# TaceoLabs/co-snarks

Measured on AMD Instinct MI355X. Metric: BN254 G1 MSM points/sec, higher is better.
Workload: dtype i32x9 29-bit-limb lazy Montgomery, i64 accumulate (BN254 Fq 254-bit); 1 GPU; BN254 G1 Pippenger MSM, uniform scalars / known-dlog points, 2^20 points per GPU (BASELINE config 2); points_total=1048576, points_per_gpu=1048576, split=single GPU, exchange_mode=none, rccl_ranks_seen=0, spinup_steps=190

## Files before the change

co-snarks_amd/csrc/curve_quad.hpp:

```cpp
#pragma once
#include <stddef.h>

#include "curve_lazy.hpp"

namespace csh {

#if defined(__HIP_DEVICE_COMPILE__) || defined(__HIPCC__)

template <int P0, int P1, int P2, int P3>
struct QuadCtrl {
  static constexpr int value = P0 | (P1 << 2) | (P2 << 4) | (P3 << 6);
};

template <int CTRL>
__device__ __forceinline__ int32_t quad_mov(int32_t v) {
  return __builtin_amdgcn_mov_dpp(v, CTRL, 0xf, 0xf, true);
}

template <int CTRL, class LP, class F32>
__device__ __forceinline__ FpS<LP, F32> quad_perm(const FpS<LP, F32>& a) {
  FpS<LP, F32> r;
#pragma unroll
  for (int i = 0; i < FpS<LP, F32>::NL; ++i) r.l[i] = quad_mov<CTRL>(a.l[i]);
  return r;
// ... 41 lines not shown
  (&p->x)[role] = q.v;
  if (role == 0) p->empty = q.empty;
}
static_assert(offsetof(XYZZLazy<Fq29s>, y) == sizeof(Fq29s) && offsetof(XYZZLazy<Fq29s>, zzz) == 3 * sizeof(Fq29s), "XYZZLazy members must be contiguous");

template <int SRC>
__device__ __forceinline__ bool quad_bcast_flag(bool f) {
  return quad_mov<QuadCtrl<SRC, SRC, SRC, SRC>::value>((int32_t)f) != 0;
}

template <class L>
__device__ __forceinline__ void qdbl(QPt<L>& acc, int role) {
  if (acc.empty) return;
  if (quad_bcast_flag<1>(acc.v.maybe_zero())) {
    if (quad_bcast_flag<1>(acc.v.is_zero_slow())) {
      acc = qpt_inf<L>();
      return;
    }
  }
  const L U = L::add(acc.v, acc.v).normalized();
  const L A = lane_select(role == 1, U, acc.v);
  const L SQ = L::sqr(A);
  const L V = quad_perm<QBcast1::value>(SQ);
  const L R2 = L::mul(A, V);
  const L M = L::add(L::add(SQ, SQ), SQ).normalized();
  const L W = quad_perm<QBcast1::value>(R2);
  const L R3 = L::mul(lane_select(role == 0, M, acc.v), lane_select(role == 0, M, W));
  const L x3 = L::sub(R3, L::add(R2, R2)).normalized();
  const L T = L::sub(R2, x3);
  const L Mb = quad_perm<QBcast0::value>(M);
  const L Tb = quad_perm<QBcast0::value>(T);
  const L y3 = L::mul_sub(Mb, Tb, R2, acc.v);
  acc.v = role == 0 ? x3 : (role == 1 ? y3 : (role == 2 ? R2 : R3));
}

template <class L>
__device__ __forceinline__ void qadd(QPt<L>& acc, const QPt<L>& p, int role) {
  if (p.empty) return;
  if (acc.empty) {
    acc = p;
    return;
  }
  const L R1 = L::mul(acc.v, quad_perm<QZzOwn::value>(p.v));
  const L R2 = L::mul(p.v, quad_perm<QZzOwn::value>(acc.v));
  const L D = L::sub(R2, R1);
  if (quad_bcast_flag<0>(D.maybe_zero())) {
    if (quad_bcast_flag<0>(D.is_zero_slow())) {
      if (quad_bcast_flag<1>(D.is_zero())) {
        qdbl<L>(acc, role);
      } else {
        acc = qpt_inf<L>();
      }
      return;
    }
  }
  const L SQ = L::sqr(D);
  const L pp = quad_perm<QBcast0::value>(SQ);
  const L pb = quad_perm<QBcast0::value>(D);
  const L R4 = L::mul(lane_select(role == 3, pb, R1), pp);
  const L ppp = quad_perm<QBcast3::value>(R4);
  const L rr = quad_perm<QBcast1::value>(SQ);
  const L x3 = L::sub(L::sub(rr, ppp), L::add(R4, R4)).normalized();
  const L T = quad_perm<QBcast0::value>(L::sub(R4, x3));
  const L a = lane_select(role == 1, D, R1);
  const L b = lane_select(role == 1, T, R4);
  const L c = lane_select(role == 1, R1, L::zero());
  const L R5 = L::mul_sub(a, b, c, ppp);
  acc.v = role == 0 ? x3 : (role == 2 ? R4 : R5);
}

template <class L>
__device__ __forceinline__ QPt<L> qmul_small(const QPt<L>& p, uint32_t k, int role) {
  QPt<L> r = qpt_inf<L>();
  if (k == 0 || p.empty) return r;
  int top = 31;
  while (!((k >> top) & 1)) --top;
  for (int b = top; b >= 0; --b) {
    qdbl<L>(r, role);
    if ((k >> b) & 1) qadd<L>(r, p, role);
  }
  return r;
}

#endif

}
```

co-snarks_amd/csrc/host_fp64.hpp:

```cpp
#pragma once
#include <stdint.h>
#include <string.h>

#include "field.hpp"

namespace csh {

template <class P>
struct Fp64 {
  static_assert(P::N % 2 == 0, "limb count must be even");
  static constexpr int N = P::N / 2;
  using Params = P;
  uint64_t l[N];

  static uint64_t word(const uint32_t* w, int i) { return (uint64_t)w[2 * i] | ((uint64_t)w[2 * i + 1] << 32); }
  static uint64_t inv64() {
    static const uint64_t v = [] {
      const uint64_t p0 = word(P::MOD, 0);
      uint64_t y = p0;
      for (int i = 0; i < 6; ++i) y *= 2 - p0 * y;
      return (uint64_t)0 - y;
    }();
    return v;
  }
  static Fp64 zero() {
    Fp64 r;
    for (int i = 0; i < N; ++i) r.l[i] = 0;
    return r;
  }
  static Fp64 one() {
    Fp64 r;
    for (int i = 0; i < N; ++i) r.l[i] = word(P::R1, i);
    return r;
  }
  bool is_zero() const {
    uint64_t a = 0;
    for (int i = 0; i < N; ++i) a |= l[i];
    return a == 0;
  }
  bool operator==(const Fp64& b) const { return memcmp(l, b.l, sizeof l) == 0; }
  bool operator!=(const Fp64& b) const { return !(*this == b); }

  static bool geq_mod(const uint64_t* a) {
    for (int i = N - 1; i >= 0; --i) {
      const uint64_t m = word(P::MOD, i);
      if (a[i] > m) return true;
      if (a[i] < m) return false;
    }
    return true;
  }
  static void sub_mod(uint64_t* a) {
    unsigned __int128 br = 0;
    for (int i = 0; i < N; ++i) {
      const unsigned __int128 d = (unsigned __int128)a[i] - word(P::MOD, i) - (uint64_t)br;
      a[i] = (uint64_t)d;
      br = (d >> 64) & 1;
    }
  }
  static Fp64 add(const Fp64& a, const Fp64& b) {
    Fp64 r;
    unsigned __int128 c = 0;
    for (int i = 0; i < N; ++i) {
      c += (unsigned __int128)a.l[i] + b.l[i];
      r.l[i] = (uint64_t)c;
      c >>= 64;
    }
    if (geq_mod(r.l)) sub_mod(r.l);
    return r;
  }
  static Fp64 sub(const Fp64& a, const Fp64& b) {
    Fp64 r;
    uint64_t br = 0;
    for (int i = 0; i < N; ++i) {
      const unsigned __int128 d = (unsigned __int128)a.l[i] - b.l[i] - br;
      r.l[i] = (uint64_t)d;
      br = (uint64_t)(d >> 64) & 1;
    }
    if (br) {
      unsigned __int128 c = 0;
      for (int i = 0; i < N; ++i) {
        c += (unsigned __int128)r.l[i] + word(P::MOD, i);
        r.l[i] = (uint64_t)c;
        c >>= 64;
      }
    }
    return r;
  }
  static Fp64 neg(const Fp64& a) { return a.is_zero() ? a : sub(zero(), a); }
  static Fp64 mul(const Fp64& a, const Fp64& b) {
    uint64_t t[N + 2];
    for (int i = 0; i < N + 2; ++i) t[i] = 0;
    const uint64_t inv = inv64();
    for (int i = 0; i < N; ++i) {
      unsigned __int128 c = 0;
      for (int j = 0; j < N; ++j) {
        c += (unsigned __int128)a.l[j] * b.l[i] + t[j];
        t[j] = (uint64_t)c;
        c >>= 64;
      }
      c += t[N];
      t[N] = (uint64_t)c;
      t[N + 1] = (uint64_t)(c >> 64);
      const uint64_t m = t[0] * inv;
      c = (unsigned __int128)m * word(P::MOD, 0) + t[0];
      c >>= 64;
      for (int j = 1; j < N; ++j) {
        c += (unsigned __int128)m * word(P::MOD, j) + t[j];
        t[j - 1] = (uint64_t)c;
        c >>= 64;
      }
      c += t[N];
      t[N - 1] = (uint64_t)c;
      t[N] = t[N + 1] + (uint64_t)(c >> 64);
    }
    Fp64 r;
    for (int i = 0; i < N; ++i) r.l[i] = t[i];
    if (t[N] || geq_mod(r.l)) sub_mod(r.l);
    return r;
  }
  static Fp64 sqr(const Fp64& a) { return mul(a, a); }
  static Fp64 mul2(const Fp64& a) { return add(a, a); }
  static Fp64 mul3(const Fp64& a) { return add(add(a, a), a); }
  static Fp64 mul4(const Fp64& a) { return mul2(mul2(a)); }
  static Fp64 mul8(const Fp64& a) { return mul2(mul4(a)); }
  static Fp64 inv(const Fp64& a) {
    Fp64 r = one();
    for (int i = P::N * 32 - 1; i >= 0; --i) {
      r = sqr(r);
      if ((P::PM2[i >> 5] >> (i & 31)) & 1) r = mul(r, a);
    }
    return r;
  }
};

template <class F>
struct Host64;
template <class P>
struct Host64<Fp<P>> {
  using type = Fp64<P>;
};
template <class P, int NR>
struct Host64<Fp2T<Fp<P>, NR>> {
  using type = Fp2T<Fp64<P>, NR>;
};

}
```

co-snarks_amd/csrc/msm_impl.hpp:

```cpp
#pragma once
#include <stdlib.h>
#include <string.h>

#include <algorithm>
#include <type_traits>
#include <vector>

#include "common.hpp"
#include "curve.hpp"
#include "curve_lazy.hpp"
#include "curve_quad.hpp"
#include "curve_pair.hpp"
#include "host_fp64.hpp"
#include "msm_digits.hpp"
#include "msm_plan.hpp"
#include "msm_sort.hpp"
#include "msm_sort_wide.hpp"


namespace csh {

struct Bn254G1Cfg { using Fq = Bn254Fq;   using Fr = Bn254Fr; static constexpr bool LAZY = true;  using L = Fq29s; static constexpr bool INLINE_ADD = true; static constexpr bool PAIR = false; };
struct Bn254G2Cfg { using Fq = Bn254Fq2;  using Fr = Bn254Fr; static constexpr bool LAZY = true;  using L = Fq29s2; static constexpr bool INLINE_ADD = true; static constexpr bool PAIR = true; static constexpr bool PAIR_ACC_DEFAULT = false; using LP = Fp2Pair<Fq29s>; };
struct Bls381G1Cfg { using Fq = Bls381Fq;  using Fr = Bls381Fr; static constexpr bool LAZY = true;  using L = Fq28s; static constexpr bool INLINE_ADD = true; static constexpr bool PAIR = false; };
// ... 117 lines not shown
          if (pos + 2 < hi) e_next2 = so[pos + 2];
        } else {
          e_next = so[pos + 1];
          pt_next = bases[e_next & 0x7fffffffu];
        }
      }
      const bool inf = stored_is_inf(pt);
      const L x = L::unpack(pt.x);
      const L y = L::unpack(pt.y).cneg_unpacked(e >> 31);
      if (pos == next) {
        pw[b + k] = acc;
        do { ++b; next = st[b + 1]; } while (next <= pos);
        acc.x = x;
        acc.y = y;
        acc.zz = L::one();
        acc.zzz = L::one();
        acc.empty = inf;
        continue;
      }
      if (inf) continue;
      lazy_madd<L, Affine<Fq>>(acc, x, y, bases + (e & 0x7fffffffu), e >> 31);
    }
    pw[b + k] = acc;
  }
}

template <class Cfg>
__global__ __launch_bounds__(ACC_BLK) void k_msm_accum_pair(const Affine<typename Cfg::Fq>* __restrict__ bases, MsmParams p,
                                                            const uint32_t* __restrict__ start, const uint32_t* __restrict__ nlanes,
                                                            const uint32_t* __restrict__ sorted, LazyPt<Cfg>* partial, uint32_t* giant_count) {
  using Fq = typename Cfg::Fq;
  using L = typename Cfg::LP;
  using LF = typename L::Base;
  using F32 = decltype(bases->x.c0);
  const int w = blockIdx.y;
  const int role = pair_role();
  const uint32_t k = (blockIdx.x * blockDim.x + threadIdx.x) >> 1;
  if (blockIdx.x == 0 && threadIdx.x == 0 && w == 0) {
    giant_count[0] = 0;
    giant_count[1] = 0;
  }
  if (k >= nlanes[w]) return;
  const uint32_t* st = start + (size_t)w * (p.NB + 2);
  const uint32_t total = st[p.NB + 1];
  const uint32_t Lw = lane_len(p, w);
  const uint32_t lo = k * Lw;
  uint32_t hi = lo + Lw;
  if (hi > total) hi = total;
  uint32_t b = upper_bound_u32(st, 1, p.NB + 1, lo) - 1;
  uint32_t next = st[b + 1];
  const uint32_t* so = sorted + (size_t)w * p.n;
  LazyPt<Cfg>* pw = partial + (size_t)w * p.tmax;
  const F32* half = reinterpret_cast<const F32*>(bases) + role;
  XYZZLazy<L> acc = XYZZLazy<L>::inf();
  uint32_t e_next = so[lo];
  F32 x_next = half[4 * (size_t)(e_next & 0x7fffffffu)], y_next = half[4 * (size_t)(e_next & 0x7fffffffu) + 2];
  for (uint32_t pos = lo; pos < hi; ++pos) {
    const uint32_t e = e_next;
    const F32 xs = x_next, ys = y_next;
    if (pos + 1 < hi) {
      e_next = so[pos + 1];
      x_next = half[4 * (size_t)(e_next & 0x7fffffffu)];
      y_next = half[4 * (size_t)(e_next & 0x7fffffffu) + 2];
    }
    const bool inf = pair_all((top_word(xs) | top_word(ys)) == 0 && xs.is_zero() && ys.is_zero());
    const L x{LF::unpack(xs)};
    const L y{LF::unpack(ys).cneg_unpacked(e >> 31)};
    if (pos == next) {
      pair_store(&pw[b + k], role, acc);
      do { ++b; next = st[b + 1]; } while (next <= pos);
      acc.x = x;
      acc.y = y;
      acc.zz = L::one();
      acc.zzz = L::one();
      acc.empty = inf;
      continue;
    }
    if (inf) continue;
    lazy_madd<L, Affine<Fq>>(acc, x, y, bases + (e & 0x7fffffffu), e >> 31);
  }
  pair_store(&pw[b + k], role, acc);
}

constexpr int TAIL_BLK = 64;
constexpr int TAIL_Q = TAIL_BLK / 4;

constexpr uint32_t MERGE_CAP = 16;
constexpr uint32_t GIANT_BIG = 256, GIANT_SLICES = 16, GIANT_BIG_CAP = 128, GIANT_ROWS = 32, GIANT_SLICED_FLAG = 0x80000000u;
__device__ __forceinline__ void giant_enqueue(uint32_t* giant_count, uint32_t* giant_list, uint32_t* big_list, uint32_t w, uint32_t b, uint32_t nparts) {
  uint32_t tag = w;
  if (nparts >= GIANT_BIG) {
    const uint32_t q = atomicAdd(giant_count + 1, 1u);
    if (q < GIANT_BIG_CAP) {
      big_list[2 * q] = w;
      big_list[2 * q + 1] = b;
      tag |= GIANT_SLICED_FLAG;
    }
  }
  const uint32_t g = atomicAdd(giant_count, 1u);
  giant_list[2 * g] = tag;
  giant_list[2 * g + 1] = b;
}
template <class Cfg>
__global__ __launch_bounds__(TAIL_BLK) void k_msm_merge(MsmParams p, const uint32_t* __restrict__ start,
                                                        const LazyPt<Cfg>* __restrict__ partial, LazyPt<Cfg>* dense,
                                                        uint32_t* giant_count, uint32_t* giant_list, uint32_t* big_list) {
  using L = typename Cfg::L;
  const int w = blockIdx.y;
  const int role = threadIdx.x & 3;
  const uint32_t b = blockIdx.x * TAIL_Q + (threadIdx.x >> 2) + 1;
  if (b > p.NB) return;
  const uint32_t* st = start + (size_t)w * (p.NB + 2);
  const uint32_t lo = st[b], hi = st[b + 1];
  QPt<L> acc = qpt_inf<L>();
  if (hi > lo) {
    const uint32_t Lw = lane_len(p, w);
    const uint32_t k0 = lo / Lw, k1 = (hi - 1) / Lw;
    const LazyPt<Cfg>* pw = partial + (size_t)w * p.tmax + b;
    if (k1 - k0 >= MERGE_CAP) {
      if (role == 0) giant_enqueue(giant_count, giant_list, big_list, (uint32_t)w, b, k1 - k0 + 1);
    } else {
      acc = qpt_load<L>(&pw[k0], role);
      for (uint32_t k = k0 + 1; k <= k1; ++k) qadd<L>(acc, qpt_load<L>(&pw[k], role), role);
    }
  }
  qpt_store<L>(&dense[(size_t)w * (p.NB + 1) + b], role, acc);
}

template <class L>
__device__ __forceinline__ void quad_block_tree(QPt<L>& x, XYZZLazy<L>* sh, int q, int nq, int role) {
  for (int half = nq >> 1; half >= 1; half >>= 1) {
    if (q >= half && q < 2 * half) qpt_store<L>(&sh[q - half], role, x);
    __syncthreads();
    if (q < half) qadd<L>(x, qpt_load<L>(&sh[q], role), role);
    __syncthreads();
  }
}

template <class Cfg>
__global__ __launch_bounds__(256) void k_msm_giant_slices(MsmParams p, const uint32_t* __restrict__ start, const LazyPt<Cfg>* __restrict__ partial,
                                                          const uint32_t* __restrict__ giant_count, const uint32_t* __restrict__ big_list,
                                                          LazyPt<Cfg>* gscratch) {
  using L = typename Cfg::L;
  __shared__ XYZZLazy<L> sh[32];
  const uint32_t sl = blockIdx.x;
  const uint32_t nbig = giant_count[1] < GIANT_BIG_CAP ? giant_count[1] : GIANT_BIG_CAP;
  const int role = threadIdx.x & 3, qd = threadIdx.x >> 2;
  for (uint32_t q = blockIdx.y; q < nbig; q += gridDim.y) {
    const uint32_t w = big_list[2 * q], b = big_list[2 * q + 1];
    const uint32_t* st = start + (size_t)w * (p.NB + 2);
    const uint32_t Lw = lane_len(p, (int)w);
    const uint32_t k0 = st[b] / Lw, k1 = (st[b + 1] - 1) / Lw;
    const uint32_t per = (k1 - k0 + GIANT_SLICES) / GIANT_SLICES;
    const uint32_t a = k0 + sl * per;
    uint32_t e = a + per;
    if (e > k1 + 1) e = k1 + 1;
    const LazyPt<Cfg>* pw = partial + (size_t)w * p.tmax + b;
    QPt<L> acc = qpt_inf<L>();
    for (uint32_t k = a + qd; k < e; k += 64) qadd<L>(acc, qpt_load<L>(&pw[k], role), role);
    quad_block_tree<L>(acc, sh, qd, 64, role);
    if (qd == 0) qpt_store<L>(&gscratch[(size_t)q * GIANT_SLICES + sl], role, acc);
  }
}

template <class Cfg>
__global__ __launch_bounds__(256) void k_msm_merge_giant(MsmParams p, const uint32_t* __restrict__ start,
                                                         const LazyPt<Cfg>* __restrict__ partial, LazyPt<Cfg>* dense,
                                                         const uint32_t* __restrict__ giant_count, const uint32_t* __restrict__ giant_list,
                                                         const uint32_t* __restrict__ big_list, const LazyPt<Cfg>* __restrict__ gscratch) {
  using L = typename Cfg::L;
  __shared__ XYZZLazy<L> sh[32];
  __shared__ uint32_t slot;
  const uint32_t count = giant_count[0];
  const uint32_t nbig = giant_count[1] < GIANT_BIG_CAP ? giant_count[1] : GIANT_BIG_CAP;
  const int role = threadIdx.x & 3, q = threadIdx.x >> 2;
  for (uint32_t g = blockIdx.x; g < count; g += gridDim.x) {
    const uint32_t tag = giant_list[2 * g], w = tag & ~GIANT_SLICED_FLAG, b = giant_list[2 * g + 1];
    QPt<L> acc = qpt_inf<L>();
    if (tag & GIANT_SLICED_FLAG) {
      __syncthreads();
      if (threadIdx.x == 0) slot = GIANT_BIG_CAP;
      __syncthreads();
      if (threadIdx.x < nbig && big_list[2 * threadIdx.x] == w && big_list[2 * threadIdx.x + 1] == b) slot = threadIdx.x;
      __syncthreads();
      if (slot < GIANT_BIG_CAP) {
        if ((uint32_t)q < GIANT_SLICES) acc = qpt_load<L>(&gscratch[(size_t)slot * GIANT_SLICES + q], role);
      } else {
        const uint32_t* st = start + (size_t)w * (p.NB + 2);
        const uint32_t Lw = lane_len(p, (int)w);
        const uint32_t k0 = st[b] / Lw, k1 = (st[b + 1] - 1) / Lw;
        const LazyPt<Cfg>* pw = partial + (size_t)w * p.tmax + b;
        for (uint32_t k = k0 + q; k <= k1; k += 64) qadd<L>(acc, qpt_load<L>(&pw[k], role), role);
      }
    } else {
      const uint32_t* st = start + (size_t)w * (p.NB + 2);
      const uint32_t Lw = lane_len(p, (int)w);
      const uint32_t k0 = st[b] / Lw, k1 = (st[b + 1] - 1) / Lw;
      const LazyPt<Cfg>* pw = partial + (size_t)w * p.tmax + b;
      for (uint32_t k = k0 + q; k <= k1; k += 64) qadd<L>(acc, qpt_load<L>(&pw[k], role), role);
    }
    quad_block_tree<L>(acc, sh, q, 64, role);
    if (q == 0) qpt_store<L>(&dense[(size_t)w * (p.NB + 1) + b], role, acc);
  }
}

template <class Cfg>
__global__ __launch_bounds__(256) void k_msm_mark_giant(MsmParams p, const uint32_t* __restrict__ start, uint32_t* giant_count, uint32_t* giant_list,
                                                        uint32_t* big_list) {
  const int w = blockIdx.y;
  const uint32_t b = blockIdx.x * 256 + threadIdx.x + 1;
  if (b > p.NB) return;
  const uint32_t* st = start + (size_t)w * (p.NB + 2);
  const uint32_t lo = st[b], hi = st[b + 1];
  const uint32_t Lw = lane_len(p, w);
  if (hi > lo && (hi - 1) / Lw - lo / Lw >= MERGE_CAP) giant_enqueue(giant_count, giant_list, big_list, (uint32_t)w, b, (hi - 1) / Lw - lo / Lw + 1);
}
template <class Cfg>
__device__ __forceinline__ QPt<typename Cfg::L> qbucket_merged(uint32_t Lw, const uint32_t* __restrict__ st, const LazyPt<Cfg>* __restrict__ pw,
                                                               const LazyPt<Cfg>* __restrict__ dw, uint32_t t, int role) {
  using L = typename Cfg::L;
  const uint32_t lo = st[t], hi = st[t + 1];
  if (hi <= lo) return qpt_inf<L>();
  const uint32_t k0 = lo / Lw, k1 = (hi - 1) / Lw;
  if (k1 - k0 >= MERGE_CAP) return qpt_load<L>(&dw[t], role);
  QPt<L> acc = qpt_load<L>(&pw[t + k0], role);
  for (uint32_t k = k0 + 1; k <= k1; ++k) qadd<L>(acc, qpt_load<L>(&pw[t + k], role), role);
  return acc;
}
template <class Cfg>
__device__ __forceinline__ XYZZLazy<typename Cfg::LP> pbucket_merged(uint32_t Lw, const uint32_t* __restrict__ st, const LazyPt<Cfg>* __restrict__ pw,
                                                                     const LazyPt<Cfg>* __restrict__ dw, uint32_t t, int role) {
  using L = typename Cfg::LP;
  const uint32_t lo = st[t], hi = st[t + 1];
  if (hi <= lo) return XYZZLazy<L>::inf();
  const uint32_t k0 = lo / Lw, k1 = (hi - 1) / Lw;
  if (k1 - k0 >= MERGE_CAP) return dw[t].empty ? XYZZLazy<L>::inf() : pair_load(&dw[t], role);
  XYZZLazy<L> acc = pw[t + k0].empty ? XYZZLazy<L>::inf() : pair_load(&pw[t + k0], role);
  for (uint32_t k = k0 + 1; k <= k1; ++k) {
    if (pw[t + k].empty) continue;
    const XYZZLazy<L> q = pair_load(&pw[t + k], role);
    lazy_add_inl<L>(acc, q);
  }
  return acc;
}

template <class Cfg, bool FUSED>
__global__ __launch_bounds__(256) void k_msm_reduce(MsmParams p, const LazyPt<Cfg>* __restrict__ dense,
                                                    LazyPt<Cfg>* segres, const uint32_t* __restrict__ start, const LazyPt<Cfg>* __restrict__ partial) {
  using L = typename Cfg::L;
  const int w = blockIdx.y;
  const int role = threadIdx.x & 3;
  const uint32_t k = blockIdx.x * 64 + (threadIdx.x >> 2);
  if (k >= p.S) return;
  const uint32_t per = (p.NB + p.S - 1) / p.S;
  const uint32_t t0 = 1 + k * per;
  uint32_t t1 = t0 + per;
  if (t1 > p.NB + 1) t1 = p.NB + 1;
  QPt<L> running = qpt_inf<L>(), acc = qpt_inf<L>();
  uint32_t prev_b = 0;
  if (t0 < t1) {
    const LazyPt<Cfg>* dw = dense + (size_t)w * (p.NB + 1);
    const uint32_t* st = FUSED ? start + (size_t)w * (p.NB + 2) : nullptr;
    const LazyPt<Cfg>* pw = FUSED ? partial + (size_t)w * p.tmax : nullptr;
    for (uint32_t t = t1; t-- > t0;) {
      QPt<L> pt;
      if constexpr (FUSED) pt = qbucket_merged<Cfg>(lane_len(p, w), st, pw, dw, t, role);
      else pt = qpt_load<L>(&dw[t], role);
      if (pt.empty) continue;
      uint32_t gap = prev_b ? prev_b - t : 0;
      if (gap) {
        if (gap <= 4) {
          while (gap--) qadd<L>(acc, running, role);
        } else {
          const QPt<L> m = qmul_small<L>(running, gap, role);
          qadd<L>(acc, m, role);
        }
      }
      qadd<L>(running, pt, role);
      prev_b = t;
    }
    if (prev_b) {
      const QPt<L> m = qmul_small<L>(running, prev_b, role);
      qadd<L>(acc, m, role);
    }
  }
  qpt_store<L>(&segres[(size_t)w * p.S + k], role, acc);
}

constexpr int RED_BLK = 256;

template <class Cfg>
__global__ __launch_bounds__(RED_BLK) void k_msm_reduce_serial(MsmParams p, const LazyPt<Cfg>* __restrict__ dense, LazyPt<Cfg>* segres) {
  using L = typename Cfg::L;
  const int w = blockIdx.y;
  const uint32_t k = blockIdx.x * RED_BLK + threadIdx.x;
  if (k >= p.S) return;
  const uint32_t per = (p.NB + p.S - 1) / p.S;
  const uint32_t t0 = 1 + k * per;
  uint32_t t1 = t0 + per;
  if (t1 > p.NB + 1) t1 = p.NB + 1;
  LazyPt<Cfg> running = LazyPt<Cfg>::inf(), acc = LazyPt<Cfg>::inf();
  uint32_t prev_b = 0;
  if (t0 < t1) {
    const LazyPt<Cfg>* dw = dense + (size_t)w * (p.NB + 1);
    for (uint32_t t = t1; t-- > t0;) {
      const LazyPt<Cfg> pt = dw[t];
      if (pt.empty) continue;
      uint32_t gap = prev_b ? prev_b - t : 0;
      if (gap) {
        if (gap <= 4) {
          while (gap--) lazy_add_inl<L>(acc, running);
        } else {
          const LazyPt<Cfg> m = lazy_mul_small<L, true>(running, gap);
          lazy_add_inl<L>(acc, m);
        }
      }
      lazy_add_inl<L>(running, pt);
      prev_b = t;
    }
    if (prev_b) {
      const LazyPt<Cfg> m = lazy_mul_small<L, true>(running, prev_b);
      lazy_add_inl<L>(acc, m);
    }
  }
  segres[(size_t)w * p.S + k] = acc;
}

template <class Cfg, bool FUSED>
__global__ __launch_bounds__(RED_BLK) void k_msm_reduce_pair(MsmParams p, const LazyPt<Cfg>* __restrict__ dense, LazyPt<Cfg>* segres,
                                                             const uint32_t* __restrict__ start, const LazyPt<Cfg>* __restrict__ partial) {
  using L = typename Cfg::LP;
  const int w = blockIdx.y;
  const int role = pair_role();
  const uint32_t k = blockIdx.x * (RED_BLK / 2) + (threadIdx.x >> 1);
  if (k >= p.S) return;
  const uint32_t per = (p.NB + p.S - 1) / p.S;
  const uint32_t t0 = 1 + k * per;
  uint32_t t1 = t0 + per;
  if (t1 > p.NB + 1) t1 = p.NB + 1;
  XYZZLazy<L> running = XYZZLazy<L>::inf(), acc = XYZZLazy<L>::inf();
  uint32_t prev_b = 0;
  if (t0 < t1) {
    const LazyPt<Cfg>* dw = dense + (size_t)w * (p.NB + 1);
    const uint32_t* st = FUSED ? start + (size_t)w * (p.NB + 2) : nullptr;
    const LazyPt<Cfg>* pw = FUSED ? partial + (size_t)w * p.tmax : nullptr;
    for (uint32_t t = t1; t-- > t0;) {
      XYZZLazy<L> pt;
      if constexpr (FUSED) {
        pt = pbucket_merged<Cfg>(lane_len(p, w), st, pw, dw, t, role);
        if (pt.empty) continue;
      } else {
        if (dw[t].empty) continue;
        pt = pair_load(&dw[t], role);
      }
      uint32_t gap = prev_b ? prev_b - t : 0;
      if (gap) {
        if (gap <= 4) {
          while (gap--) lazy_add_inl<L>(acc, running);
        } else {
          const XYZZLazy<L> m = lazy_mul_small<L, true>(running, gap);
          lazy_add_inl<L>(acc, m);
        }
      }
      lazy_add_inl<L>(running, pt);
      prev_b = t;
// ... 146 lines not shown
  CSH_TRY(msm_sort_prepare<Fr>(p, pdig, scalars_dev, st, ar, &ss));
  CSH_TRY(msm_sort_launch(p, ss.sb, st, ev));
  *out = SortOut{ss.sb.start, ss.sb.nlanes, ss.sb.sorted};
  return CSH_OK;
}

template <class Cfg>
struct BucketBufs {
  LazyPt<Cfg>*partial, *segres, *dense, *fold_a, *fold_b;
  uint32_t* giant;
  uint32_t* big;
  LazyPt<Cfg>* gscratch;
  uint32_t fold_n1, max_lanes, max_giant, giant_blocks;
};
constexpr int MAX_GROUPS = 8;
template <class Cfg>
BucketBufs<Cfg> bucket_take(const MsmParams& p, Arena& ar) {
  BucketBufs<Cfg> b;
  b.max_lanes = (uint32_t)(((size_t)p.n + p.L - 1) / p.L);
  b.max_giant = (uint32_t)(((uint64_t)b.max_lanes * p.W) / MERGE_CAP + 1);
  b.giant_blocks = b.max_giant < 1024 ? b.max_giant : 1024;
  b.partial = ar.take<LazyPt<Cfg>>((size_t)p.tmax * p.W);
  b.segres = ar.take<LazyPt<Cfg>>((size_t)p.S * p.W);
  b.dense = ar.take<LazyPt<Cfg>>((size_t)(p.NB + 1) * p.W);
  b.giant = ar.take<uint32_t>((2 * (size_t)b.max_giant + 2) * MAX_GROUPS);
  b.big = ar.take<uint32_t>((size_t)2 * GIANT_BIG_CAP * MAX_GROUPS);
  b.gscratch = ar.take<LazyPt<Cfg>>((size_t)GIANT_BIG_CAP * GIANT_SLICES * MAX_GROUPS);
  b.fold_n1 = (p.S + 127) / 128;
  b.fold_a = ar.take<LazyPt<Cfg>>((size_t)b.fold_n1 * p.W);
  b.fold_b = ar.take<LazyPt<Cfg>>((size_t)b.fold_n1 * p.W);
  return b;
}
template <class Cfg>
size_t msm_bucket_bytes(const MsmParams* pp) {
  Arena sizing;
  bucket_take<Cfg>(*pp, sizing);
  return sizing.off;
}

template <class Cfg>
int bucket_group(const void* points, const MsmParams& p_all, const SortOut& so, const BucketBufs<Cfg>& bb, int w0, int nw, int group, hipStream_t st,
                 void* win_out_dev, hipEvent_t* ev) {
  using Fq = typename Cfg::Fq;
  MsmParams p = p_all;
  p.wide = p_all.wide > w0 ? p_all.wide - w0 : 0;
  const size_t len = (size_t)p.NB + 2;
  const uint32_t* start = so.start + len * w0;
  const uint32_t* nlanes = so.nlanes + w0;
  const uint32_t* sorted = so.sorted + (size_t)p.n * w0;
  LazyPt<Cfg>* partial = bb.partial + (size_t)p.tmax * w0;
  LazyPt<Cfg>* segres = bb.segres + (size_t)p.S * w0;
  LazyPt<Cfg>* dense = bb.dense + (size_t)(p.NB + 1) * w0;
  LazyPt<Cfg>* fold_a = bb.fold_a + (size_t)bb.fold_n1 * w0;
  LazyPt<Cfg>* fold_b = bb.fold_b + (size_t)bb.fold_n1 * w0;
  uint32_t* giant = bb.giant + (2 * (size_t)bb.max_giant + 2) * group;
  uint32_t* big = bb.big + (size_t)2 * GIANT_BIG_CAP * group;
  LazyPt<Cfg>* gscratch = bb.gscratch + (size_t)GIANT_BIG_CAP * GIANT_SLICES * group;
  const Affine<Fq>* bases = reinterpret_cast<const Affine<Fq>*>(points);
  {
    const int tb = tune().acc_blk.load(std::memory_order_relaxed);
    const int blk = (tb == 64 || tb == 128) ? tb : ACC_BLK;
    bool pair = false;
    if constexpr (Cfg::PAIR) pair = Cfg::PAIR_ACC_DEFAULT != ((tune().msm_variant.load(std::memory_order_relaxed) & 2) != 0);
    if constexpr (Cfg::PAIR) {
      if (pair) {
        const dim3 ag((2 * bb.max_lanes + blk - 1) / blk, nw), ab(blk);
        hipLaunchKernelGGL(k_msm_accum_pair<Cfg>, ag, ab, 0, st, bases, p, start, nlanes, sorted, partial, giant);
      }
    }
    if (!pair) {
      const dim3 ag((bb.max_lanes + blk - 1) / blk, nw), ab(blk);
      hipLaunchKernelGGL(k_msm_accum<Cfg>, ag, ab, 0, st, bases, p, start, nlanes, sorted, partial, giant);
    }
  }
  if (ev) CSH_HIP(hipEventRecord(ev[4], st));
  const int variant = tune().msm_variant.load(std::memory_order_relaxed);
  int form;
  if constexpr (Cfg::PAIR) form = (variant & 1) ? 1 : ((variant & 4) ? 0 : 2);
  else form = (variant & 1) ? 0 : 1;
  const bool fused = form != 0 && (variant & 16) != 0;
  if (fused)
    hipLaunchKernelGGL(k_msm_mark_giant<Cfg>, dim3((p.NB + 255) / 256, nw), dim3(256), 0, st, p, start, giant, giant + 2, big);
  else
    hipLaunchKernelGGL(k_msm_merge<Cfg>, dim3((p.NB + TAIL_Q - 1) / TAIL_Q, nw), dim3(TAIL_BLK), 0, st, p, start, partial, dense, giant, giant + 2, big);
  hipLaunchKernelGGL(k_msm_giant_slices<Cfg>, dim3(GIANT_SLICES, GIANT_ROWS), dim3(256), 0, st, p, start, partial, giant, big, gscratch);
  hipLaunchKernelGGL(k_msm_merge_giant<Cfg>, dim3(bb.giant_blocks), dim3(256), 0, st, p, start, partial, dense, giant, giant + 2, big, gscratch);
  MsmParams pr = p;
  if (form == 1) {
    pr.S = std::min(p.S, reduce_segments(p.NB, p.W, 4));
    if (fused) hipLaunchKernelGGL((k_msm_reduce<Cfg, true>), dim3((pr.S + 63) / 64, nw), dim3(256), 0, st, pr, dense, segres, start, partial);
    else hipLaunchKernelGGL((k_msm_reduce<Cfg, false>), dim3((pr.S + 63) / 64, nw), dim3(256), 0, st, pr, dense, segres, start, partial);
  } else if (form == 2) {
    pr.S = std::min(p.S, reduce_segments(p.NB, p.W, 2));
    if constexpr (Cfg::PAIR) {
      if (fused) hipLaunchKernelGGL((k_msm_reduce_pair<Cfg, true>), dim3((pr.S + RED_BLK / 2 - 1) / (RED_BLK / 2), nw), dim3(RED_BLK), 0, st, pr, dense, segres, start, partial);
      else hipLaunchKernelGGL((k_msm_reduce_pair<Cfg, false>), dim3((pr.S + RED_BLK / 2 - 1) / (RED_BLK / 2), nw), dim3(RED_BLK), 0, st, pr, dense, segres, start, partial);
    }
  } else {
    hipLaunchKernelGGL(k_msm_reduce_serial<Cfg>, dim3((pr.S + RED_BLK - 1) / RED_BLK, nw), dim3(RED_BLK), 0, st, pr, dense, segres);
  }
  const LazyPt<Cfg>* cur = segres;
  uint32_t cur_n = pr.S, cur_stride = pr.S;
  LazyPt<Cfg>* nxt = fold_a;
  XYZZ<Fq>* win_out = reinterpret_cast<XYZZ<Fq>*>(win_out_dev) + w0;
  bool exported = false;
  while (cur_n > 1) {
    const uint32_t out_n = (cur_n + 127) / 128;
    exported = out_n == 1;
    hipLaunchKernelGGL(k_msm_fold_tree<Cfg>, dim3(out_n, nw), dim3(256), 0, st, cur, cur_stride, cur_n, nxt, bb.fold_n1,
                       exported ? win_out : (XYZZ<Fq>*)nullptr);
    cur = nxt;
    cur_n = out_n;
    cur_stride = bb.fold_n1;
    nxt = nxt == fold_a ? fold_b : fold_a;
  }
  if (!exported)
    hipLaunchKernelGGL(k_msm_gather_windows<Cfg>, dim3(1), dim3(MAX_WINDOWS), 0, st, cur, cur_stride, nw, win_out);
  CSH_HIP(hipGetLastError());
  return CSH_OK;
}

template <class Cfg>
int msm_bucket_stage(const void* points, const MsmParams* pp, const SortOut* so, hipStream_t st, Arena* arp, void* win_out_dev, hipEvent_t* ev) {
  const MsmParams& p = *pp;
  const BucketBufs<Cfg> bb = bucket_take<Cfg>(p, *arp);
  CSH_TRY((bucket_group<Cfg>(points, p, *so, bb, 0, p.W, 0, st, win_out_dev, ev)));
  if (ev) CSH_HIP(hipEventRecord(ev[5], st));
  return CSH_OK;
}


inline bool msm_use_table(const Bases* B, size_t n) {
  if (!B->table || n == 0 || tune().msm_no_table.load(std::memory_order_relaxed)) return false;
  if ((uint64_t)n * (uint64_t)B->table_W >= (uint64_t(1) << 31) || (uint64_t)B->n * (uint64_t)B->table_W >= (uint64_t(1) << 31)) return false;
  return n * 8 >= B->n;
}

template <class Cfg>
int accum_occupancy() {
  static std::atomic<int> cache{0};
  int v = cache.load(std::memory_order_relaxed);
  if (v) return v;
  v = 1;
  if constexpr (!Cfg::PAIR) {
    int blocks = 0;
    if (hipOccupancyMaxActiveBlocksPerMultiprocessor(&blocks, k_msm_accum<Cfg>, ACC_BLK, 0) == hipSuccess && blocks > 0) {
      v = blocks * (ACC_BLK / 64) / 4;
      v = v < 1 ? 1 : (v > 8 ? 8 : v);
    }
  }
  cache.store(v, std::memory_order_relaxed);
  return v;
}

template <class Cfg>
int msm_windows_dev(const Bases* B, size_t offset, size_t n, const uint64_t* scalars_dev, int mont, hipStream_t st,
                    XYZZ<typename Cfg::Fq>* win_out_dev , MsmParams* p_out) {
  using Fr = typename Cfg::Fr;
  using Fq = typename Cfg::Fq;
  const MsmTable table{B->table_c, B->table_W, B->n, offset};
  const MsmPlan plan = msm_plan(n, Fr::Params::BITS, mont, accum_occupancy<Cfg>(), msm_use_table(B, n) ? &table : nullptr);
  const MsmParams &p = plan.srt, &pdig = plan.dig;
  const void* points = plan.merged ? B->table : reinterpret_cast<const Affine<Fq>*>(B->points) + offset;
  msm_record_params(p);
  *p_out = p;
  Arena& ar = arena_for(st);
  CSH_TRY(ar.reserve(msm_sort_bytes(p, pdig) + msm_bucket_bytes<Cfg>(&p)));
// ... 343 lines not shown
```

Baseline: 651.1 million points/s.

## Compact long merges in-block, use 2-bit window scalar mult, speed host field math

New measurement: 668.2 million points/s (median of 6 runs). 2.6% higher.

```diff
diff --git a/co-snarks_amd/csrc/curve_quad.hpp b/co-snarks_amd/csrc/curve_quad.hpp
--- a/co-snarks_amd/csrc/curve_quad.hpp
+++ b/co-snarks_amd/csrc/curve_quad.hpp
@@ -147,6 +147,30 @@
   return r;
 }
 
+template <class L>
+__device__ __forceinline__ QPt<L> qmul_small_w2(const QPt<L>& p, uint32_t k, int role) {
+  QPt<L> r = qpt_inf<L>();
+  if (k == 0 || p.empty) return r;
+  QPt<L> p2 = p;
+  qdbl<L>(p2, role);
+  QPt<L> p3 = p2;
+  qadd<L>(p3, p, role);
+  int top = 30;
+  while (!((k >> top) & 3)) top -= 2;
+  for (int s = top; s >= 0; s -= 2) {
+    qdbl<L>(r, role);
+    qdbl<L>(r, role);
+    const uint32_t d = (k >> s) & 3;
+    if (d) {
+      QPt<L> o;
+      o.v = lane_select(d == 1, p.v, lane_select(d == 2, p2.v, p3.v));
+      o.empty = d == 1 ? p.empty : (d == 2 ? p2.empty : p3.empty);
+      qadd<L>(r, o, role);
+    }
+  }
+  return r;
+}
+
 #endif
 
 }
diff --git a/co-snarks_amd/csrc/host_fp64.hpp b/co-snarks_amd/csrc/host_fp64.hpp
--- a/co-snarks_amd/csrc/host_fp64.hpp
+++ b/co-snarks_amd/csrc/host_fp64.hpp
@@ -4,25 +4,49 @@
 
 #include "field.hpp"
 
+#if defined(__clang__)
+#define CSH_HOST_UNROLL _Pragma("unroll")
+#elif defined(__GNUC__)
+#define CSH_HOST_UNROLL _Pragma("GCC unroll 16")
+#else
+#define CSH_HOST_UNROLL
+#endif
+
 namespace csh {
+
+template <int N>
+struct Fp64Consts {
+  uint64_t mod[N], one[N], pm2[N];
+  uint64_t inv;
+};
+template <class P>
+constexpr Fp64Consts<P::N / 2> fp64_consts() {
+  Fp64Consts<P::N / 2> k{};
+  for (int i = 0; i < P::N / 2; ++i) {
+    k.mod[i] = (uint64_t)P::MOD[2 * i] | ((uint64_t)P::MOD[2 * i + 1] << 32);
+    k.one[i] = (uint64_t)P::R1[2 * i] | ((uint64_t)P::R1[2 * i + 1] << 32);
+    k.pm2[i] = (uint64_t)P::PM2[2 * i] | ((uint64_t)P::PM2[2 * i + 1] << 32);
+  }
+  uint64_t y = k.mod[0];
+  for (int i = 0; i < 6; ++i) y *= 2 - k.mod[0] * y;
+  k.inv = (uint64_t)0 - y;
+  return k;
+}
 
 template <class P>
 struct Fp64 {
   static_assert(P::N % 2 == 0, "limb count must be even");
   static constexpr int N = P::N / 2;
   using Params = P;
+  using u128 = unsigned __int128;
   uint64_t l[N];
 
+  static constexpr Fp64Consts<N> K = fp64_consts<P>();
+  static_assert((K.mod[N - 1] >> 63) == 0 && K.mod[N - 1] != 0x7fffffffffffffffull, "the modulus must leave its top bit free");
+  static_assert((uint64_t)(K.mod[0] * K.inv) == ~(uint64_t)0, "inv must be -p^-1 mod 2^64");
+
   static uint64_t word(const uint32_t* w, int i) { return (uint64_t)w[2 * i] | ((uint64_t)w[2 * i + 1] << 32); }
-  static uint64_t inv64() {
-    static const uint64_t v = [] {
-      const uint64_t p0 = word(P::MOD, 0);
-      uint64_t y = p0;
-      for (int i = 0; i < 6; ++i) y *= 2 - p0 * y;
-      return (uint64_t)0 - y;
-    }();
-    return v;
-  }
+  static constexpr uint64_t inv64() { return K.inv; }
   static Fp64 zero() {
     Fp64 r;
     for (int i = 0; i < N; ++i) r.l[i] = 0;
@@ -30,7 +54,7 @@
   }
   static Fp64 one() {
     Fp64 r;
-    for (int i = 0; i < N; ++i) r.l[i] = word(P::R1, i);
+    for (int i = 0; i < N; ++i) r.l[i] = K.one[i];
     return r;
   }
   bool is_zero() const {
@@ -42,26 +66,28 @@
   bool operator!=(const Fp64& b) const { return !(*this == b); }
 
   static bool geq_mod(const uint64_t* a) {
+    CSH_HOST_UNROLL
     for (int i = N - 1; i >= 0; --i) {
-      const uint64_t m = word(P::MOD, i);
-      if (a[i] > m) return true;
-      if (a[i] < m) return false;
+      if (a[i] > K.mod[i]) return true;
+      if (a[i] < K.mod[i]) return false;
     }
     return true;
   }
   static void sub_mod(uint64_t* a) {
-    unsigned __int128 br = 0;
-    for (int i = 0; i < N; ++i) {
-      const unsigned __int128 d = (unsigned __int128)a[i] - word(P::MOD, i) - (uint64_t)br;
+    u128 br = 0;
+    CSH_HOST_UNROLL
+    for (int i = 0; i < N; ++i) {
+      const u128 d = (u128)a[i] - K.mod[i] - (uint64_t)br;
       a[i] = (uint64_t)d;
       br = (d >> 64) & 1;
     }
   }
   static Fp64 add(const Fp64& a, const Fp64& b) {
     Fp64 r;
-    unsigned __int128 c = 0;
-    for (int i = 0; i < N; ++i) {
-      c += (unsigned __int128)a.l[i] + b.l[i];
+    u128 c = 0;
+    CSH_HOST_UNROLL
+    for (int i = 0; i < N; ++i) {
+      c += (u128)a.l[i] + b.l[i];
       r.l[i] = (uint64_t)c;
       c >>= 64;
     }
@@ -71,15 +97,17 @@
   static Fp64 sub(const Fp64& a, const Fp64& b) {
     Fp64 r;
     uint64_t br = 0;
-    for (int i = 0; i < N; ++i) {
-      const unsigned __int128 d = (unsigned __int128)a.l[i] - b.l[i] - br;
+    CSH_HOST_UNROLL
+    for (int i = 0; i < N; ++i) {
+      const u128 d = (u128)a.l[i] - b.l[i] - br;
       r.l[i] = (uint64_t)d;
       br = (uint64_t)(d >> 64) & 1;
     }
     if (br) {
-      unsigned __int128 c = 0;
+      u128 c = 0;
+      CSH_HOST_UNROLL
       for (int i = 0; i < N; ++i) {
-        c += (unsigned __int128)r.l[i] + word(P::MOD, i);
+        c += (u128)r.l[i] + K.mod[i];
         r.l[i] = (uint64_t)c;
         c >>= 64;
       }
@@ -87,47 +115,138 @@
     return r;
   }
   static Fp64 neg(const Fp64& a) { return a.is_zero() ? a : sub(zero(), a); }
+
   static Fp64 mul(const Fp64& a, const Fp64& b) {
-    uint64_t t[N + 2];
-    for (int i = 0; i < N + 2; ++i) t[i] = 0;
-    const uint64_t inv = inv64();
-    for (int i = 0; i < N; ++i) {
-      unsigned __int128 c = 0;
-      for (int j = 0; j < N; ++j) {
-        c += (unsigned __int128)a.l[j] * b.l[i] + t[j];
-        t[j] = (uint64_t)c;
-        c >>= 64;
-      }
-      c += t[N];
-      t[N] = (uint64_t)c;
-      t[N + 1] = (uint64_t)(c >> 64);
-      const uint64_t m = t[0] * inv;
-      c = (unsigned __int128)m * word(P::MOD, 0) + t[0];
-      c >>= 64;
+    uint64_t t[N];
+    CSH_HOST_UNROLL
+    for (int j = 0; j < N; ++j) t[j] = 0;
+    CSH_HOST_UNROLL
+    for (int i = 0; i < N; ++i) {
+      u128 A = (u128)a.l[i] * b.l[0] + t[0];
+      const uint64_t m = (uint64_t)A * K.inv;
+      u128 C = (u128)m * K.mod[0] + (uint64_t)A;
+      CSH_HOST_UNROLL
       for (int j = 1; j < N; ++j) {
-        c += (unsigned __int128)m * word(P::MOD, j) + t[j];
-        t[j - 1] = (uint64_t)c;
-        c >>= 64;
-      }
-      c += t[N];
-      t[N - 1] = (uint64_t)c;
-      t[N] = t[N + 1] + (uint64_t)(c >> 64);
-    }
-    Fp64 r;
+        A = (u128)a.l[i] * b.l[j] + t[j] + (uint64_t)(A >> 64);
+        C = (u128)m * K.mod[j] + (uint64_t)A + (uint64_t)(C >> 64);
+        t[j - 1] = (uint64_t)C;
+      }
+      t[N - 1] = (uint64_t)(A >> 64) + (uint64_t)(C >> 64);
+    }
+    Fp64 r;
+    CSH_HOST_UNROLL
     for (int i = 0; i < N; ++i) r.l[i] = t[i];
-    if (t[N] || geq_mod(r.l)) sub_mod(r.l);
-    return r;
-  }
-  static Fp64 sqr(const Fp64& a) { return mul(a, a); }
+    if (geq_mod(r.l)) sub_mod(r.l);
+    return r;
+  }
+  static Fp64 sqr(const Fp64& a) {
+    uint64_t t[2 * N];
+    CSH_HOST_UNROLL
+    for (int j = 0; j < 2 * N; ++j) t[j] = 0;
+    CSH_HOST_UNROLL
+    for (int i = 0; i < N - 1; ++i) {
+      uint64_t c = 0;
+      CSH_HOST_UNROLL
+      for (int j = i + 1; j < N; ++j) {
+        const u128 v = (u128)a.l[i] * a.l[j] + t[i + j] + c;
+        t[i + j] = (uint64_t)v;
+        c = (uint64_t)(v >> 64);
+      }
+      t[i + N] = c;
+    }
+    CSH_HOST_UNROLL
+    for (int j = 2 * N - 1; j > 0; --j) t[j] = (t[j] << 1) | (t[j - 1] >> 63);
+    t[0] = 0;
+    {
+      uint64_t c = 0;
+      CSH_HOST_UNROLL
+      for (int i = 0; i < N; ++i) {
+        const u128 d = (u128)a.l[i] * a.l[i];
+        const u128 lo = (u128)t[2 * i] + (uint64_t)d + c;
+        t[2 * i] = (uint64_t)lo;
+        const u128 hi = (u128)t[2 * i + 1] + (uint64_t)(d >> 64) + (uint64_t)(lo >> 64);
+        t[2 * i + 1] = (uint64_t)hi;
+        c = (uint64_t)(hi >> 64);
+      }
+    }
+    uint64_t top = 0;
+    CSH_HOST_UNROLL
+    for (int i = 0; i < N; ++i) {
+      const uint64_t m = t[i] * K.inv;
+      u128 C = (u128)m * K.mod[0] + t[i];
+      CSH_HOST_UNROLL
+      for (int j = 1; j < N; ++j) {
+        C = (u128)m * K.mod[j] + t[i + j] + (uint64_t)(C >> 64);
+        t[i + j] = (uint64_t)C;
+      }
+      const u128 s = (u128)t[i + N] + (uint64_t)(C >> 64) + top;
+      t[i + N] = (uint64_t)s;
+      top = (uint64_t)(s >> 64);
+    }
+    Fp64 r;
+    CSH_HOST_UNROLL
+    for (int i = 0; i < N; ++i) r.l[i] = t[i + N];
+    if (geq_mod(r.l)) sub_mod(r.l);
+    return r;
+  }
   static Fp64 mul2(const Fp64& a) { return add(a, a); }
   static Fp64 mul3(const Fp64& a) { return add(add(a, a), a); }
   static Fp64 mul4(const Fp64& a) { return mul2(mul2(a)); }
   static Fp64 mul8(const Fp64& a) { return mul2(mul4(a)); }
   static Fp64 inv(const Fp64& a) {
+    Fp64 pw[16];
+    pw[0] = one();
+    pw[1] = a;
+    for (int i = 2; i < 16; ++i) pw[i] = (i & 1) ? mul(pw[i - 1], a) : sqr(pw[i / 2]);
+    Fp64 r = one();
+    bool started = false;
+    for (int i = 16 * N - 1; i >= 0; --i) {
+      const unsigned d = (unsigned)(K.pm2[i >> 4] >> (4 * (i & 15))) & 15u;
+      if (started) r = sqr(sqr(sqr(sqr(r))));
+      if (d) {
+        r = started ? mul(r, pw[d]) : pw[d];
+        started = true;
+      }
+    }
+    return r;
+  }
+
+  static Fp64 mul_looped(const Fp64& a, const Fp64& b) {
+    uint64_t t[N + 2];
+    for (int i = 0; i < N + 2; ++i) t[i] = 0;
+    const uint64_t inv = K.inv;
+    for (int i = 0; i < N; ++i) {
+      u128 c = 0;
+      for (int j = 0; j < N; ++j) {
+        c += (u128)a.l[j] * b.l[i] + t[j];
+        t[j] = (uint64_t)c;
+        c >>= 64;
+      }
+      c += t[N];
+      t[N] = (uint64_t)c;
+      t[N + 1] = (uint64_t)(c >> 64);
+      const uint64_t m = t[0] * inv;
+      c = (u128)m * K.mod[0] + t[0];
+      c >>= 64;
+      for (int j = 1; j < N; ++j) {
+        c += (u128)m * K.mod[j] + t[j];
+        t[j - 1] = (uint64_t)c;
+        c >>= 64;
+      }
+      c += t[N];
+      t[N - 1] = (uint64_t)c;
+      t[N] = t[N + 1] + (uint64_t)(c >> 64);
+    }
+    Fp64 r;
+    for (int i = 0; i < N; ++i) r.l[i] = t[i];
+    if (t[N] || geq_mod(r.l)) sub_mod(r.l);
+    return r;
+  }
+  static Fp64 inv_looped(const Fp64& a) {
     Fp64 r = one();
     for (int i = P::N * 32 - 1; i >= 0; --i) {
-      r = sqr(r);
-      if ((P::PM2[i >> 5] >> (i & 31)) & 1) r = mul(r, a);
+      r = mul_looped(r, r);
+      if ((P::PM2[i >> 5] >> (i & 31)) & 1) r = mul_looped(r, a);
     }
     return r;
   }
diff --git a/co-snarks_amd/csrc/msm_impl.hpp b/co-snarks_amd/csrc/msm_impl.hpp
--- a/co-snarks_amd/csrc/msm_impl.hpp
+++ b/co-snarks_amd/csrc/msm_impl.hpp
@@ -223,8 +223,8 @@
   pair_store(&pw[b + k], role, acc);
 }
 
-constexpr int TAIL_BLK = 64;
-constexpr int TAIL_Q = TAIL_BLK / 4;
+constexpr int MERGE_BLK = 256;
+constexpr int MERGE_Q = MERGE_BLK / 4;
 
 constexpr uint32_t MERGE_CAP = 16;
 constexpr uint32_t GIANT_BIG = 256, GIANT_SLICES = 16, GIANT_BIG_CAP = 128, GIANT_ROWS = 32, GIANT_SLICED_FLAG = 0x80000000u;
@@ -243,29 +243,45 @@
   giant_list[2 * g + 1] = b;
 }
 template <class Cfg>
-__global__ __launch_bounds__(TAIL_BLK) void k_msm_merge(MsmParams p, const uint32_t* __restrict__ start,
-                                                        const LazyPt<Cfg>* __restrict__ partial, LazyPt<Cfg>* dense,
-                                                        uint32_t* giant_count, uint32_t* giant_list, uint32_t* big_list) {
+__global__ __launch_bounds__(MERGE_BLK) void k_msm_merge(MsmParams p, const uint32_t* __restrict__ start,
+                                                         const LazyPt<Cfg>* __restrict__ partial, LazyPt<Cfg>* dense,
+                                                         uint32_t* giant_count, uint32_t* giant_list, uint32_t* big_list) {
   using L = typename Cfg::L;
+  __shared__ uint32_t list_n;
+  __shared__ uint32_t list[MERGE_Q];
   const int w = blockIdx.y;
   const int role = threadIdx.x & 3;
-  const uint32_t b = blockIdx.x * TAIL_Q + (threadIdx.x >> 2) + 1;
-  if (b > p.NB) return;
+  const uint32_t q = threadIdx.x >> 2;
+  const uint32_t b0 = blockIdx.x * MERGE_Q + 1;
   const uint32_t* st = start + (size_t)w * (p.NB + 2);
-  const uint32_t lo = st[b], hi = st[b + 1];
-  QPt<L> acc = qpt_inf<L>();
-  if (hi > lo) {
-    const uint32_t Lw = lane_len(p, w);
-    const uint32_t k0 = lo / Lw, k1 = (hi - 1) / Lw;
-    const LazyPt<Cfg>* pw = partial + (size_t)w * p.tmax + b;
-    if (k1 - k0 >= MERGE_CAP) {
-      if (role == 0) giant_enqueue(giant_count, giant_list, big_list, (uint32_t)w, b, k1 - k0 + 1);
-    } else {
-      acc = qpt_load<L>(&pw[k0], role);
-      for (uint32_t k = k0 + 1; k <= k1; ++k) qadd<L>(acc, qpt_load<L>(&pw[k], role), role);
-    }
-  }
-  qpt_store<L>(&dense[(size_t)w * (p.NB + 1) + b], role, acc);
+  const uint32_t Lw = lane_len(p, w);
+  const LazyPt<Cfg>* pw = partial + (size_t)w * p.tmax;
+  LazyPt<Cfg>* dw = dense + (size_t)w * (p.NB + 1);
+  if (threadIdx.x == 0) list_n = 0;
+  __syncthreads();
+  if (const uint32_t b = b0 + q; b <= p.NB) {
+    const uint32_t lo = st[b], hi = st[b + 1];
+    QPt<L> acc = qpt_inf<L>();
+    if (hi > lo) {
+      const uint32_t k0 = lo / Lw, k1 = (hi - 1) / Lw;
+      if (k1 - k0 >= MERGE_CAP) {
+        if (role == 0) giant_enqueue(giant_count, giant_list, big_list, (uint32_t)w, b, k1 - k0 + 1);
+      } else {
+        acc = qpt_load<L>(&pw[b + k0], role);
+        if (k1 > k0) qadd<L>(acc, qpt_load<L>(&pw[b + k0 + 1], role), role);
+        if (k1 - k0 >= 2 && role == 0) list[atomicAdd(&list_n, 1u)] = q;
+      }
+    }
+    qpt_store<L>(&dw[b], role, acc);
+  }
+  __syncthreads();
+  if (q < list_n) {
+    const uint32_t b = b0 + list[q];
+    const uint32_t k0 = st[b] / Lw, k1 = (st[b + 1] - 1) / Lw;
+    QPt<L> acc = qpt_load<L>(&dw[b], role);
+    for (uint32_t k = k0 + 2; k <= k1; ++k) qadd<L>(acc, qpt_load<L>(&pw[b + k], role), role);
+    qpt_store<L>(&dw[b], role, acc);
+  }
 }
 
 template <class L>
@@ -413,7 +429,7 @@
         if (gap <= 4) {
           while (gap--) qadd<L>(acc, running, role);
         } else {
-          const QPt<L> m = qmul_small<L>(running, gap, role);
+          const QPt<L> m = qmul_small_w2<L>(running, gap, role);
           qadd<L>(acc, m, role);
         }
       }
@@ -421,7 +437,7 @@
       prev_b = t;
     }
     if (prev_b) {
-      const QPt<L> m = qmul_small<L>(running, prev_b, role);
+      const QPt<L> m = qmul_small_w2<L>(running, prev_b, role);
       qadd<L>(acc, m, role);
     }
   }
@@ -734,7 +750,7 @@
   if (fused)
     hipLaunchKernelGGL(k_msm_mark_giant<Cfg>, dim3((p.NB + 255) / 256, nw), dim3(256), 0, st, p, start, giant, giant + 2, big);
   else
-    hipLaunchKernelGGL(k_msm_merge<Cfg>, dim3((p.NB + TAIL_Q - 1) / TAIL_Q, nw), dim3(TAIL_BLK), 0, st, p, start, partial, dense, giant, giant + 2, big);
+    hipLaunchKernelGGL(k_msm_merge<Cfg>, dim3((p.NB + MERGE_Q - 1) / MERGE_Q, nw), dim3(MERGE_BLK), 0, st, p, start, partial, dense, giant, giant + 2, big);
   hipLaunchKernelGGL(k_msm_giant_slices<Cfg>, dim3(GIANT_SLICES, GIANT_ROWS), dim3(256), 0, st, p, start, partial, giant, big, gscratch);
   hipLaunchKernelGGL(k_msm_merge_giant<Cfg>, dim3(bb.giant_blocks), dim3(256), 0, st, p, start, partial, dense, giant, giant + 2, big, gscratch);
   MsmParams pr = p;
```
